# ds4dm/Tulip.jl

Measured on AMD Instinct MI355X. Metric: IPM Newton-step rate: KKT.update! (A*D*A'+Rd, supernodal Cholesky) + 4 KKT.solve!, higher is better.
Workload: dtype f64

## Files before the change

### tulip.jl_amd/csrc/kernels.hip

```cpp
#include <hip/hip_runtime.h>

#include <cstdlib>
#include <mutex>

#include "tlpk_device.hpp"

namespace tlpk {


typedef double v4f64 __attribute__((ext_vector_type(4)));
__device__ __forceinline__ double readlane_f64(const double v, const int l) {
    const int lo = __builtin_amdgcn_readlane(__double2loint(v), l), hi = __builtin_amdgcn_readlane(__double2hiint(v), l);
    return __hiloint2double(hi, lo);
}

__device__ __forceinline__ double *front_u(const DevCtx &c, const FrontDesc &fd) {
    return (fd.ubuf ? c.U1 : c.U0) + fd.uoff;
}
__device__ __forceinline__ double *pcol(const DevCtx &c, const FrontDesc &fd, i32 col) { return c.Lval + fd.loff + pk_off(fd.lda, col); }
__device__ __forceinline__ i32 pld(const FrontDesc &fd, i32 col) { return fd.lda - ((col >> 6) << 6); }

__global__ void k_compute_d(i64 n, const double *__restrict__ theta, const double *__restrict__ regP,
                            double *__restrict__ D) {
    const i64 j = (i64)blockIdx.x * blockDim.x + threadIdx.x;
// ... 1910 lines not shown
                any |= valid[a][b];
            }
    }
    v4f64 acc[CA][4];
#pragma unroll
    for (int a = 0; a < CA; ++a)
#pragma unroll
        for (int b = 0; b < 4; ++b) acc[a][b] = (v4f64){0.0, 0.0, 0.0, 0.0};

    const int lr = lane & 15, lk = lane >> 4;
    const int sr = tid & 127, sk0 = tid >> 7;
    const i32 ra = t.i0 + sr, rb_ = t.j0 + sr;
    const bool raok = FULL || (ra < f), rbok = FULL || ((rb_ < f) && !diag_tile);
    const int sk0u = __builtin_amdgcn_readfirstlane(sk0);
    double pa[UPD_NLD], pb[UPD_NLD];

    auto load_slab = [&](i32 kk, bool full_k) {
        if (FULL && full_k) {
#pragma unroll
            for (int it = 0; it < UPD_NLD; ++it) {
                const double *Pk = P + pk_off(lda, t.k0 + kk + sk0u + KS * it);
                pa[it] = Pk[ra];
                pb[it] = Pk[rb_];
                if (SIGNED) pb[it] *= sgk[kk + sk0 + KS * it];
            }
        } else {
#pragma unroll
            for (int it = 0; it < UPD_NLD; ++it) {
                const bool kok = (kk + sk0u + KS * it) < t.kw;
                const double *Pk = P + pk_off(lda, t.k0 + min(kk + sk0u + KS * it, t.kw - 1));
                pa[it] = (kok && raok) ? Pk[ra] : 0.0;
                pb[it] = (kok && rbok) ? Pk[rb_] : 0.0;
                if (SIGNED) pb[it] *= sgk[min(kk + sk0 + KS * it, t.kw - 1)];
            }
        }
    };
    auto store_slab = [&](int buf) {
#pragma unroll
        for (int it = 0; it < UPD_NLD; ++it) {
            const int k = sk0 + KS * it;
            As[buf][k * UPD_LD + sr] = pa[it];
            if (FULL || !diag_tile) Bs[buf][k * UPD_LD + sr] = pb[it];
        }
    };

    const i32 *segp = t.seg ? c.upd_seg + (t.seg - 1) : nullptr;
    if (segp || t.kw >= 2 * UPD_KT) {
        unsigned voa = (unsigned)min(t.i0 + sr, f - 1) * 8u, vob = (unsigned)min(t.j0 + sr, f - 1) * 8u;
        const char *Pc = reinterpret_cast<const char *>(P);
        const i32 nseg = __builtin_amdgcn_readfirstlane(segp ? segp[0] : 1);
        i32 k_slab = __builtin_amdgcn_readfirstlane(segp ? segp[1] : t.k0);
        i32 k_rem = __builtin_amdgcn_readfirstlane(segp ? segp[2] : (t.kw / UPD_KT));
        i32 k_seg = 0;
        const char *sb[UPD_NLD];
#pragma unroll
        for (int it = 0; it < UPD_NLD; ++it) sb[it] = Pc + pk_off(lda, k_slab + sk0u + KS * it) * 8;
        i64 step = (i64)UPD_KT * 8 * (lda - ((k_slab >> 6) << 6));
        auto ld_a = [&]() {
            asm volatile("" : "+v"(voa));
#pragma unroll
            for (int it = 0; it < UPD_NLD; ++it) pa[it] = *reinterpret_cast<const double *>(sb[it] + voa);
        };
        const double *sgf = SIGNED ? c.csign + fd.col0 : nullptr;
        auto ld_b = [&]() {
            asm volatile("" : "+v"(vob));
#pragma unroll
            for (int it = 0; it < UPD_NLD; ++it) {
                pb[it] = *reinterpret_cast<const double *>(sb[it] + vob);
                if (SIGNED) pb[it] *= sgf[k_slab + sk0 + KS * it];
            }
            k_slab += UPD_KT;
            const bool cross = (k_slab & 63) == 0;
#pragma unroll
            for (int it = 0; it < UPD_NLD; ++it) sb[it] += step - (cross ? (i64)(64 * 8) * (sk0u + KS * it + 1) : 0);
            step -= cross ? 64 * 8 * UPD_KT : 0;
            if (__builtin_expect(--k_rem == 0, 0)) {
                if (++k_seg < nseg) {
                    k_slab = __builtin_amdgcn_readfirstlane(segp[1 + 2 * k_seg]);
                    k_rem = __builtin_amdgcn_readfirstlane(segp[2 + 2 * k_seg]);
#pragma unroll
                    for (int it = 0; it < UPD_NLD; ++it) sb[it] = Pc + pk_off(lda, k_slab + sk0u + KS * it) * 8;
                    step = (i64)UPD_KT * 8 * (lda - ((k_slab >> 6) << 6));
                }
            }
        };
        auto st_ab = [&](int buf) {
#pragma unroll
            for (int it = 0; it < UPD_NLD; ++it) {
                As[buf][(sk0 + KS * it) * UPD_LD + sr] = pa[it];
                Bs[buf][(sk0 + KS * it) * UPD_LD + sr] = pb[it];
            }
        };
        auto mfma_round = [&](int buf, auto &&hook) {
            const double *At = As[buf] + wr * 64 + lr + lk * UPD_LD;
            const double *Bt = Bs[buf] + wc * WCW + lr + lk * UPD_LD;
#pragma unroll
            for (int k4 = 0; k4 < UPD_KT; k4 += 4) {
                double av[CA], bv[4];
                if (any) {
#pragma unroll
                    for (int a = 0; a < CA; ++a) av[a] = Bt[k4 * UPD_LD + a * 16];
#pragma unroll
                    for (int b = 0; b < 4; ++b) bv[b] = At[k4 * UPD_LD + b * 16];
                }
                hook(k4);
                if (any) {
#pragma unroll
                    for (int a = 0; a < CA; ++a)
#pragma unroll
                        for (int b = 0; b < 4; ++b)
                            acc[a][b] = __builtin_amdgcn_mfma_f64_16x16x4f64(av[a], bv[b], acc[a][b], 0, 0, 0);
                }
            }
        };
        int cur = 0;
        const i32 nrounds = segp ? t.nsl : t.kw / UPD_KT;
        const bool dma_ok = UPD_DMA && !SIGNED && ((fd.loff | (i64)lda | (i64)t.i0 | (i64)t.j0) & 1) == 0;
        if (dma_ok) {
            typedef __attribute__((address_space(3))) double upd_lds_double;
            const unsigned la_a0 = (unsigned)__builtin_amdgcn_readfirstlane((int)(unsigned)(unsigned long long)(upd_lds_double *)&As[0][0]);
            const unsigned la_b0 = (unsigned)__builtin_amdgcn_readfirstlane((int)(unsigned)(unsigned long long)(upd_lds_double *)&Bs[0][0]);
            constexpr unsigned BUFB = UPD_KT * UPD_LD * 8;
            constexpr int CPW = UPD_KT / NW;
            unsigned dva = (unsigned)min(t.i0 + 2 * lane, lda - 2) * 8u, dvb = (unsigned)min(t.j0 + 2 * lane, lda - 2) * 8u;
            const char *db[CPW];
#pragma unroll
            for (int e = 0; e < CPW; ++e) db[e] = Pc + pk_off(lda, k_slab + wave + NW * e) * 8;
            auto dma_slab = [&](const int buf) {
                asm volatile("" : "+v"(dva), "+v"(dvb));
#pragma unroll
                for (int e = 0; e < CPW; ++e) {
                    const unsigned ko = (unsigned)(wave + NW * e) * (unsigned)(UPD_LD * 8) + (unsigned)buf * BUFB;
                    asm volatile("s_mov_b32 m0, %0\n\ts_nop 0\n\tglobal_load_lds_dwordx4 %1, %2" :: "s"(la_a0 + ko), "v"(dva), "s"(db[e]) : "memory", "m0");
                    asm volatile("s_mov_b32 m0, %0\n\ts_nop 0\n\tglobal_load_lds_dwordx4 %1, %2" :: "s"(la_b0 + ko), "v"(dvb), "s"(db[e]) : "memory", "m0");
                }
                k_slab += UPD_KT;
                const bool cross = (k_slab & 63) == 0;
#pragma unroll
                for (int e = 0; e < CPW; ++e) db[e] += step - (cross ? (i64)(64 * 8) * (wave + NW * e + 1) : 0);
                step -= cross ? 64 * 8 * UPD_KT : 0;
                if (__builtin_expect(--k_rem == 0, 0)) {
                    if (++k_seg < nseg) {
                        k_slab = __builtin_amdgcn_readfirstlane(segp[1 + 2 * k_seg]);
                        k_rem = __builtin_amdgcn_readfirstlane(segp[2 + 2 * k_seg]);
#pragma unroll
                        for (int e = 0; e < CPW; ++e) db[e] = Pc + pk_off(lda, k_slab + wave + NW * e) * 8;
                        step = (i64)UPD_KT * 8 * (lda - ((k_slab >> 6) << 6));
                    }
                }
            };
            dma_slab(0);
            asm volatile("s_waitcnt vmcnt(0)" ::: "memory");
            __syncthreads();
            for (i32 rd = 0; rd < nrounds; ++rd) {
                const bool have_next = rd + 1 < nrounds;
                mfma_round(cur, [&](int k4) {
                    if (k4 == 0 && have_next) dma_slab(cur ^ 1);
                });
                asm volatile("s_waitcnt vmcnt(0)" ::: "memory");
                __syncthreads();
                cur ^= 1;
            }
        } else {
        ld_a(); ld_b();
        st_ab(0);
        ld_a(); ld_b();
        __syncthreads();
#ifdef UPD_TRACE
        if (threadIdx.x == 0) ((unsigned long long *)c.spart)[(size_t)blockIdx.x * 8 + 1] = wall_clock64();
#endif
        for (i32 rd = 0; rd < nrounds; ++rd) {
            const bool have_next = rd + 1 < nrounds, have_next2 = rd + 2 < nrounds;
            mfma_round(cur, [&](int k4) {
                if (k4 == 0 && have_next) st_ab(cur ^ 1);
                if (k4 == 4 && have_next2) ld_a();
                if (k4 == 8 && have_next2) ld_b();
            });
            __syncthreads();
            cur ^= 1;
        }
        }
        if (t.kw % UPD_KT) {
            const i32 kk = (t.kw / UPD_KT) * UPD_KT;
#pragma unroll
            for (int it = 0; it < UPD_NLD; ++it) {
                const bool kok = (kk + sk0u + KS * it) < t.kw;
                const double *Pk = P + pk_off(lda, t.k0 + min(kk + sk0u + KS * it, t.kw - 1));
                pa[it] = kok ? *reinterpret_cast<const double *>(reinterpret_cast<const char *>(Pk) + voa) : 0.0;
                pb[it] = kok ? *reinterpret_cast<const double *>(reinterpret_cast<const char *>(Pk) + vob) : 0.0;
                if (SIGNED) pb[it] *= sgk[min(kk + sk0 + KS * it, t.kw - 1)];
            }
            st_ab(cur);
            __syncthreads();
            mfma_round(cur, [](int) {});
        }
        goto epilogue;
    }
    {
    load_slab(0, UPD_KT <= t.kw);
    store_slab(0);
    __syncthreads();
    int cur = 0;
    for (i32 kk = 0; kk < t.kw; kk += UPD_KT) {
        const bool more = (kk + UPD_KT) < t.kw;
#if defined(UPD_VARIANT) && (UPD_VARIANT == 1 || UPD_VARIANT == 6)
        if (more && kk < 0) load_slab(kk + UPD_KT, true);
#else
        if (more) load_slab(kk + UPD_KT, (kk + 2 * UPD_KT) <= t.kw);
#endif
        if (any) {
            const double *At = As[cur] + wr * 64 + lr + lk * UPD_LD;
            const double *Bt = (diag_tile ? As[cur] : Bs[cur]) + wc * WCW + lr + lk * UPD_LD;
#pragma unroll
            for (int k4 = 0; k4 < UPD_KT; k4 += 4) {
                double av[CA], bv[4];
#pragma unroll
                for (int a = 0; a < CA; ++a) av[a] = Bt[k4 * UPD_LD + a * 16];
#pragma unroll
                for (int b = 0; b < 4; ++b) bv[b] = At[k4 * UPD_LD + b * 16];
#pragma unroll
                for (int a = 0; a < CA; ++a)
#pragma unroll
                    for (int b = 0; b < 4; ++b) {
                        if constexpr (FULL) {
                            acc[a][b] = __builtin_amdgcn_mfma_f64_16x16x4f64(av[a], bv[b], acc[a][b], 0, 0, 0);
                        } else {
                            if (valid[a][b]) acc[a][b] = __builtin_amdgcn_mfma_f64_16x16x4f64(av[a], bv[b], acc[a][b], 0, 0, 0);
                        }
                    }
            }
        }
        if (more) store_slab(cur ^ 1);
#if !(defined(UPD_VARIANT) && (UPD_VARIANT == 4 || UPD_VARIANT == 6))
        __syncthreads();
#endif
        cur ^= 1;
    }
    }
epilogue:
#ifdef UPD_TRACE
    if (threadIdx.x == 0) ((unsigned long long *)c.spart)[(size_t)blockIdx.x * 8 + 2] = wall_clock64();
#endif
    if (!any) return;
    if (t.pad1) {
        double *Sp = c.spart + (i64)(t.pad1 - 1) * (TILE * TILE);
#pragma unroll
        for (int a = 0; a < CA; ++a)
// ... 289 lines not shown

__device__ __forceinline__ bool chain_wait(const ChainItem &it, const unsigned *cnt, int *info, const int lane, const unsigned timeout_ms, const int dbg_slot) {
    const int n01 = it.n0 + it.n1, ntot = n01 + (it.w2 >= 0 ? 1 : 0);
    if (ntot == 0) return __hip_atomic_load(info + 1, __ATOMIC_RELAXED, __HIP_MEMORY_SCOPE_AGENT) == 0;
    const bool act = lane < ntot;
    const int e = min(lane, ntot - 1);
    const int idx = (e < it.n0) ? it.w0 + e : ((e < n01) ? it.w1 + (e - it.n0) : it.w2);
    const unsigned need = (unsigned)((e < it.n0) ? it.need0 : ((e < n01) ? it.need1 : it.need2));
    const unsigned *p = cnt + idx;
    bool dead = false;
    unsigned spins = 0;
    const unsigned long long t0 = wall_clock64();
    unsigned v = need;
    if (act) v = __hip_atomic_load(p, __ATOMIC_RELAXED, __HIP_MEMORY_SCOPE_AGENT);
    while (!dead && !__all(v >= need)) {
        if (spins < 64u) __builtin_amdgcn_s_sleep(8);
        else if (spins < 512u) __builtin_amdgcn_s_sleep(32);
        else __builtin_amdgcn_s_sleep(127);
        if ((++spins & 63u) == 0u) {
            int flag = 0;
            if (lane == 0) flag = __hip_atomic_load(info + 1, __ATOMIC_RELAXED, __HIP_MEMORY_SCOPE_AGENT);
            if (__builtin_amdgcn_readfirstlane(flag) != 0) dead = true;
            else if (wall_clock64() - t0 > (unsigned long long)timeout_ms * 100000ull) {
                if (v < need && __hip_atomic_exchange(info + 3, 1, __ATOMIC_RELAXED, __HIP_MEMORY_SCOPE_AGENT) == 0) {
                    info[4] = dbg_slot; info[5] = it.role; info[6] = idx; info[7] = (int)need; info[8] = (int)v; info[9] = (int)blockIdx.x; info[10] = (int)gridDim.x; info[11] = it.task;
                }
                if (lane == 0) __hip_atomic_store(info + 1, 1, __ATOMIC_RELAXED, __HIP_MEMORY_SCOPE_AGENT);
                dead = true;
            }
        }
        if (act) v = __hip_atomic_load(p, __ATOMIC_RELAXED, __HIP_MEMORY_SCOPE_AGENT);
    }
    asm volatile("" ::: "memory");
    __builtin_amdgcn_fence(__ATOMIC_ACQUIRE, "agent");
    return !dead;
}


template <class T> __device__ __forceinline__ T *uni(T *p) {
    const unsigned long long v = reinterpret_cast<unsigned long long>(p);
    const unsigned lo = (unsigned)__builtin_amdgcn_readfirstlane((int)(unsigned)v), hi = (unsigned)__builtin_amdgcn_readfirstlane((int)(unsigned)(v >> 32));
    typedef __attribute__((address_space(1))) T gT;
    return (T *)(gT *)(((unsigned long long)hi << 32) | lo);
}
typedef __attribute__((address_space(3))) double lds_double;
typedef __attribute__((address_space(3))) char lds_char;
__device__ __forceinline__ double *uni_lds(lds_double *p) {
    const unsigned v = (unsigned)__builtin_amdgcn_readfirstlane((int)(unsigned)(unsigned long long)(lds_char *)p);
    return (double *)(lds_double *)(lds_char *)(unsigned long long)v;
}
__device__ __forceinline__ DevCtx uni_ctx(const DevCtx &c) {
    DevCtx u = c;
    u.fronts = uni(c.fronts); u.Lval = uni(c.Lval); u.U0 = uni(c.U0); u.U1 = uni(c.U1); u.dinv = uni(c.dinv); u.spart = uni(c.spart); u.info = uni(c.info);
    u.csign = uni(c.csign); u.upd_seg = uni(c.upd_seg);
    return u;
}

template <bool SIGNED>
__device__ __noinline__ void chain_role_update(const UpdateTask *tp_, const DevCtx &c_, lds_double *lds_) {
    const UpdateTask *tp = uni(tp_); const DevCtx c = uni_ctx(c_); double *lds = uni_lds(lds_);
    const UpdateTask t{tp->front, tp->k0, tp->kw, tp->i0, tp->j0, tp->jlim, tp->beta0, tp->pad1, tp->seg, tp->nsl, tp->pad2, 0};
    const FrontDesc fd = c.fronts[t.front];
    if (t.pad2 == 2) { update_tile32<SIGNED>(t, fd, c); return; }
    if (t.pad2) { update_tile64<SIGNED>(t, fd, c, lds); return; }
    double (*As)[UPD_KT * UPD_LD] = reinterpret_cast<double (*)[UPD_KT * UPD_LD]>(lds);
    const bool full = (t.i0 + TILE <= fd.f) && (t.j0 + TILE <= t.jlim) && (t.i0 >= t.j0 + TILE);
    if (full) update_tile<true, SIGNED, 4>(t, fd, c, As, As + 2);
    else update_tile<false, SIGNED, 4>(t, fd, c, As, As + 2);
}
template <bool SIGNED>
__device__ __noinline__ void chain_role_potrf(const PotrfTask *tp_, const DevCtx &c_, lds_double *lds_, unsigned *prog_) {
    const PotrfTask *tp = uni(tp_); const DevCtx c = uni_ctx(c_); double *lds = uni_lds(lds_);
    const PotrfTask t{tp->front, tp->k0, tp->nb, tp->kprev};
    const FrontDesc fd = c.fronts[t.front];
    potrf_wide_task<SIGNED, 3>(t, fd, c, lds, prog_ ? uni(prog_) : nullptr);
    __builtin_amdgcn_s_setprio(0);
}
template <bool SIGNED>
__device__ __noinline__ void chain_role_trsm(const TrsmTask *tp_, const DevCtx &c_, lds_double *lds_, lds_double *dyn_, unsigned *cnt_, const unsigned timeout_ms_) {
    const TrsmTask *tp = uni(tp_); const DevCtx c = uni_ctx(c_); double *lds = uni_lds(lds_);
    const TrsmTask t{tp->front, tp->k0, tp->nb, tp->row0, tp->kprev, tp->fuse_nb, tp->pad1, tp->pad2};
    const FrontDesc fd = c.fronts[t.front];
    if (t.nb == NB_OUT) {
        if constexpr (TRSM_DMA) {
            const TrsmProg pg{t.pad2 > 0 ? uni(cnt_) + (t.pad2 - 1) : nullptr, c.info, (unsigned)__builtin_amdgcn_readfirstlane((int)timeout_ms_)};
            if (dyn_) {
                if (t.pad2 > 0) trsm_task_dma<SIGNED, 4, true>(t, fd, c, lds, uni_lds(dyn_), pg);
                else trsm_task_dma<SIGNED, 4, false>(t, fd, c, lds, uni_lds(dyn_), pg);
            } else {
                if (t.pad2 > 0) trsm_task_dma<SIGNED, 2, true>(t, fd, c, lds, nullptr, pg);
                else trsm_task_dma<SIGNED, 2, false>(t, fd, c, lds, nullptr, pg);
            }
        } else trsm_task<SIGNED, true>(t, fd, c, reinterpret_cast<double (*)[NB_IN * LDW]>(lds));
    } else trsm_task<SIGNED, false>(t, fd, c, reinterpret_cast<double (*)[NB_IN * LDW]>(lds));
}
__device__ __noinline__ void chain_role_reduce(const UpdateTask *tp_, const int sub_, const DevCtx &c_) {
    const UpdateTask *tp = uni(tp_); const DevCtx c = uni_ctx(c_); const int sub = __builtin_amdgcn_readfirstlane(sub_);
    const UpdateTask t{tp->front, tp->k0, tp->kw, tp->i0, tp->j0, tp->jlim, tp->beta0, tp->pad1, tp->seg, tp->nsl, 0, 0};
    const FrontDesc fd = c.fronts[t.front];
    reduce_part(t, sub, fd, c);
}

template <bool SIGNED>
__global__ __launch_bounds__(256, 2) void k_chain(const ChainArgs a, DevCtx c) {
    __shared__ __attribute__((aligned(16))) double lds[CHAIN_LDS];
    extern __shared__ __attribute__((aligned(16))) double chain_dyn[];
    lds_double *dyn = a.dyn_lds >= 2u * TRSM_DMA_BLK * sizeof(double) ? (lds_double *)chain_dyn : (lds_double *)nullptr;
// ... 1176 lines not shown
```

### tulip.jl_amd/csrc/tlpk_api.cpp

```cpp
#include <hip/hip_runtime.h>

#include <dlfcn.h>

#include <algorithm>
#include <atomic>
#include <chrono>
#include <climits>
#include <cmath>
#include <limits>
#include <cstdio>
#include <cstdlib>
#include <cstring>
#include <new>
#include <optional>
#include <string>
#include <thread>
#include <utility>
#include <vector>
#include <condition_variable>
#include <functional>
#include <initializer_list>
#include <mutex>

#include "../../include/tlpk.h"
// ... 249 lines not shown
            for (char f : S.front_fa) any_fa |= (f != 0);
            std::vector<i64> colptr_c;
            if (!every) {
                colptr_c.assign((size_t)S.m + 1, 0);
                i64 cnt = 0;
                for (i64 kk = 0; kk < S.m; ++kk) {
                    colptr_c[(size_t)kk] = cnt;
                    for (i64 e = S.Sp[(size_t)kk]; e < S.Sp[(size_t)kk + 1]; ++e) cnt += (S.s_local[(size_t)e] != 0);
                }
                colptr_c[(size_t)S.m] = cnt;
                if (cnt != d.n_asm) { h->last_error = "assembly list: column pointers do not match the compacted entries"; return TLPK_INTERNAL; }
            }
            const std::vector<i64> &colptr = every ? S.Sp : colptr_c;
            if (any_fa) {
                std::vector<i64> tsmall;
                if (every) tsmall.assign(S.s_target.begin(), S.s_target.end()); else tsmall = tgt;
                for (i64 kk = 0; kk < S.m; ++kk)
                    if (S.front_fa[(size_t)S.sn_of_col[(size_t)kk]])
                        for (i64 q = colptr[(size_t)kk]; q < colptr[(size_t)kk + 1]; ++q) tsmall[(size_t)q] = -1;
                UP(d.asm_colptr, colptr); UP(d.asm_target_small, tsmall);
            }
            bool any = false;
            for (char f : S.front_upper) any |= (f != 0);
            d.has_upper = any;
            if (any) {
                std::vector<unsigned char> up((size_t)d.n_asm, 0);
                for (i64 kk = 0; kk < S.m; ++kk)
                    if (S.front_upper[(size_t)S.sn_of_col[(size_t)kk]]) std::fill(up.begin() + colptr[(size_t)kk], up.begin() + colptr[(size_t)kk + 1], (unsigned char)1);
                UP(d.asm_upper, up);
            }
        }
        if (every) { UP(d.asm_target, S.s_target); UP(d.asm_diag, S.s_diag_row); UP(d.asm_ptr, S.pair_ptr); }
        else { UP(d.asm_target, tgt); UP(d.asm_diag, diag); UP(d.asm_ptr, ptr); }
        if (!d.asm_target_small) d.asm_target_small = d.asm_target;
        UP(d.pair_w, S.pair_w); UP(d.pair_j, S.pair_j);
        if (np != (i64)S.pair_w.size()) { h->last_error = "assembly list compaction mismatch"; return TLPK_INTERNAL; }
    }
    const FrontDesc *fr = nullptr; const i32 *ri = nullptr, *re = nullptr, *ch = nullptr;
    { FrontDesc *p; UP(p, S.fronts); fr = p; }
    { i32 *p; UP(p, S.rowidx); ri = p; }
    { i32 *p; UP(p, S.rel); re = p; }
    { i32 *p; UP(p, S.ea_tab); d.ctx.ea_tab = p; }
    { i32 *p; UP(p, S.children); ch = p; }
    d.ctx.fronts = fr; d.ctx.rowidx = ri; d.ctx.rel = re; d.ctx.children = ch;
    { i64 *p; UP(p, S.gth_ptr); d.ctx.gth_ptr = p; }
    { i64 *p; UP(p, S.gth_src); d.ctx.gth_src = p; }
    UP(d.fa_tasks, S.fa_tasks);
    UP(d.ea_tasks, S.ea_tasks); UP(d.potrf_tasks, S.potrf_tasks); UP(d.trsm_tasks, S.trsm_tasks);
    UP(d.update_tasks, S.update_tasks); UP(d.reduce_tasks, S.reduce_tasks);
    UP(d.chain_items, S.chain_items); d.n_chain_cnt = S.chain_counters;
    if (S.chain_counters > 0 && (rc = dev_alloc(h, &d.chain_cnt, S.chain_counters)) != TLPK_OK) return rc;
    if (!S.chain_items.empty() && std::getenv("TLPK_CHAIN_TRACE") && (rc = dev_alloc(h, &d.chain_trace, 4 * (i64)S.chain_items.size())) != TLPK_OK) return rc;
    { i32 *p; UP(p, S.upd_seg); d.ctx.upd_seg = p; }
    d.n_single = (i64)S.single_col.size();
    UP(d.single_loff, S.single_loff); UP(d.single_dinvoff, S.single_dinvoff); UP(d.single_col, S.single_col);
    UP(d.zero_tasks, S.zero_tasks); d.n_zero_tasks = (i64)S.zero_tasks.size() / 2; d.n_zero_lower = d.has_upper ? S.n_zero_lower : d.n_zero_tasks;
    UP(d.zero_small, S.zero_small); d.n_zero_small = (i64)S.zero_small.size();
    UP(d.fwd_gather_tasks, S.fwd_gather_tasks); UP(d.fwd_diag_tasks, S.fwd_diag_tasks);
    UP(d.fwd_update_tasks, S.fwd_update_tasks); UP(d.bwd_update_tasks, S.bwd_update_tasks);
    UP(d.fwd_small_tasks, S.fwd_small_tasks); UP(d.bwd_small_tasks, S.bwd_small_tasks);
    UP(d.fwd_sweep_tasks, S.fwd_sweep_tasks); UP(d.bwd_sweep_tasks, S.bwd_sweep_tasks);
#undef UP
#define AL(dst, cnt) if ((rc = dev_alloc(h, &(dst), (cnt))) != TLPK_OK) return rc
    AL(d.ctx.Lval, S.lval_len); AL(d.ctx.U0, S.ubuf_len[0]); AL(d.ctx.U1, S.ubuf_len[1]);
    if (std::getenv("TLPK_POISON") && S.lval_len > 0) { HIPCHK(h, hipMemset(d.ctx.Lval, 0xFF, (size_t)S.lval_len * 8)); HIPCHK(h, hipDeviceSynchronize()); }
    AL(d.ctx.uc, 2 * S.uc_len); AL(d.ctx.xw, 2 * S.m); AL(d.ctx.info, 16);
    d.ctx.xw2 = S.m; d.ctx.uc2 = S.uc_len; AL(d.ctx.dinv, S.dinv_len); AL(d.ctx.spart, S.spart_len);
    const i64 nn = std::max<i64>(S.n + (S.n_dense > 0 ? 1 : 0), S.k2_n + 1);
    AL(h->d_theta, nn); AL(h->d_regP, nn); AL(h->d_regD, S.m); AL(h->d_D, nn);
    AL(h->d_xip, S.m); AL(h->d_xid, nn); AL(h->d_dx, nn); AL(h->d_dy, S.m);
    AL(d.rhs_w, std::max<i64>(2 * S.n, 1));
    d.asm_D = h->d_D; d.asm_regD = h->d_regD;
    HIPCHK(h, hipMemset(h->d_theta, 0, (size_t)nn * 8)); HIPCHK(h, hipMemset(h->d_regP, 0, (size_t)nn * 8)); HIPCHK(h, hipMemset(h->d_xid, 0, (size_t)nn * 8));
    HIPCHK(h, hipMemset(h->d_regD, 0, (size_t)std::max<i64>(S.m, 1) * 8)); HIPCHK(h, hipMemset(h->d_xip, 0, (size_t)std::max<i64>(S.m, 1) * 8));
    if (h->refine_steps > 0) { AL(h->d_r1, S.m); AL(h->d_r2, nn); AL(h->d_cx, nn); AL(h->d_cy, S.m); AL(h->d_ref, 8); }
    d.ctx.csign = nullptr;
    d.ctx.small_full = std::getenv("TLPK_SMALL_FULL") ? std::atoi(std::getenv("TLPK_SMALL_FULL")) : 0;
    d.ctx.upd_remap = 2;
    if (const char *e = std::getenv("TLPK_UPD_REMAP")) d.ctx.upd_remap = std::atoi(e);
    if (S.system == 1 || S.n_dense > 0) { double *p; if ((rc = dev_upload(h, &p, S.csign)) != TLPK_OK) return rc; d.ctx.csign = p; }
#undef AL
    {
        i32 nslots = 0;
        h->sweep_slot_fwd.assign(S.fwd_launches.size(), -1); h->sweep_slot_bwd.assign(S.bwd_launches.size(), -1);
        for (size_t i = 0; i < S.fwd_launches.size(); ++i) if (S.fwd_launches[i].kind == LK_FWD_SWEEP) h->sweep_slot_fwd[i] = nslots++;
        for (size_t i = 0; i < S.bwd_launches.size(); ++i) if (S.bwd_launches[i].kind == LK_BWD_SWEEP) h->sweep_slot_bwd[i] = nslots++;
        const i64 nt = ((i64)nslots + 15) / 16 * 16;
        unsigned long long *blk = nullptr;
        if ((rc = dev_alloc(h, &blk, nt + 4 * S.m)) != TLPK_OK) return rc;
        d.sweep_tickets = blk; d.sweep_xh = reinterpret_cast<double *>(blk + nt);
        d.sweep_reset_bytes = (nt + 2 * S.m) * 8; d.sweep_reset_bytes2 = (nt + 4 * S.m) * 8;
        HIPCHK(h, hipMemset(d.ctx.info, 0, 16 * sizeof(int)));
    }
    HIPCHK(h, hipHostMalloc((void **)&h->h_info, 4 * sizeof(int), hipHostMallocDefault));
    h->h_info[0] = h->h_info[1] = h->h_info[2] = h->h_info[3] = 0;
    uvec<double>().swap(S.pair_w); uvec<i32>().swap(S.pair_j);
    return TLPK_OK;
}

void find_markers(tlpk_handle *h) {
    h->factor_marker = h->S.factor_launches.size();
    h->fwd_marker = h->S.fwd_launches.size();
    for (size_t i = 0; i < h->S.factor_launches.size(); ++i)
        if (h->S.factor_launches[i].kind == LK_ALLREDUCE_ROOT) h->factor_marker = i;
    for (size_t i = 0; i < h->S.fwd_launches.size(); ++i)
        if (h->S.fwd_launches[i].kind == LK_ALLREDUCE_ROOT) h->fwd_marker = i;
}

struct GraphKey { int kind; const void *p[8]; bool operator==(const GraphKey &o) const { return kind == o.kind && std::memcmp(p, o.p, sizeof(p)) == 0; } };

inline bool graph_usable(const tlpk_handle *h) {
    return h->use_graph && !h->profile && !h->serial && (h->S.ngroups <= 1 || h->force_graph);
}

inline bool graph_usable_solve(const tlpk_handle *h) {
    static const bool on = [] { const char *e = std::getenv("TLPK_GRAPH_SOLVE"); return e && std::atoi(e) != 0; }();
    if (graph_usable(h)) return true;
    return on && h->use_graph && !h->profile && !h->serial && h->S.solve_single_stream && !h->root_pending && h->opt.nranks == 1;
}

template <class F>
int graph_or_direct(tlpk_handle *h, const GraphKey &key, F &&body, bool usable) {
    if (!usable) return body();
    for (size_t i = 0; i < h->graph_keys.size(); ++i)
        if (*reinterpret_cast<const GraphKey *>(h->graph_keys[i].data()) == key) {
            HIPCHK(h, hipGraphLaunch(h->graph_execs[i], h->stream));
            return TLPK_OK;
        }
    hipGraph_t g = nullptr;
    if (hipStreamBeginCapture(h->stream, hipStreamCaptureModeThreadLocal) != hipSuccess) { (void)hipGetLastError(); h->use_graph = false; return body(); }
    const int rc = body();
    hipGraphExec_t exec = nullptr;
// ... 226 lines not shown
    if (rc == TLPK_OK) {
        find_markers(h);
        h->nlink = (h->S.root_front >= 0) ? h->S.fronts[h->S.root_front].ns : 0;
        h->first_link = h->S.m - h->nlink;
    }
    return rc;
}

static int create_device(tlpk_handle *h, const tlpk_options &def) {
    int rc = TLPK_OK;
    if (def.device >= 0) {
        int ndev = 0;
        if (hipGetDeviceCount(&ndev) != hipSuccess || def.device >= ndev) {
            h->last_error = "no HIP device " + std::to_string(def.device) + " visible";
            return TLPK_NO_DEVICE;
        }
        h->device = def.device;
        hipError_t e = hipSetDevice(h->device);
        if (e == hipSuccess) e = hipStreamCreateWithFlags(&h->stream, hipStreamNonBlocking);
        h->gstream[0] = h->stream;
        const int ng = std::max(1, h->S.ngroups);
        for (int g = 1; g < ng && e == hipSuccess; ++g) e = hipStreamCreateWithFlags(&h->gstream[g], hipStreamNonBlocking);
        for (int g = 0; g < ng && e == hipSuccess; ++g) e = hipStreamCreateWithFlags(&h->sstream[g], hipStreamNonBlocking);
        if (e == hipSuccess) e = hipEventCreateWithFlags(&h->ev_fork, hipEventDisableTiming);
        if (e == hipSuccess && ng >= 2) {
            int least = 0, greatest = 0;
            hipDeviceGetStreamPriorityRange(&least, &greatest);
            e = hipStreamCreateWithPriority(&h->zstream, hipStreamNonBlocking, least);
        }
        if (e == hipSuccess && ng >= 2) e = hipEventCreateWithFlags(&h->ev_zfork, hipEventDisableTiming);
        if (e == hipSuccess && ng >= 2) e = hipEventCreateWithFlags(&h->ev_upper, hipEventDisableTiming);
        for (int g = 1; g < ng && e == hipSuccess; ++g) e = hipEventCreateWithFlags(&h->ev_join[g], hipEventDisableTiming);
        for (int g = 0; g < ng && e == hipSuccess; ++g) e = hipEventCreateWithFlags(&h->ev_side[g], hipEventDisableTiming);
        if (e == hipSuccess && h->stagger) e = hipEventCreateWithFlags(&h->ev_stagger, hipEventDisableTiming);
        if (e == hipSuccess) e = hipEventCreate(&h->ev0);
        if (e == hipSuccess) e = hipEventCreate(&h->ev1);
        if (e == hipSuccess && h->S.root_front >= 0 && h->opt.nranks == 1) {
            e = hipStreamCreateWithFlags(&h->rstream, hipStreamNonBlocking);
            if (e == hipSuccess) e = hipEventCreateWithFlags(&h->ev_blocks, hipEventDisableTiming);
            if (e == hipSuccess) e = hipEventCreateWithFlags(&h->ev_root, hipEventDisableTiming);
        }
        if (e != hipSuccess) rc = hip_fail(h, e, "device init");
        if (rc == TLPK_OK) {
            size_t free_b = 0, total_b = 0;
            hipMemGetInfo(&free_b, &total_b);
            const double budget = def.mem_budget_bytes > 0 ? (double)def.mem_budget_bytes : 0.9 * (double)free_b;
            const double need = 8.0 * ((double)h->S.lval_len + (double)h->S.ubuf_len[0] + (double)h->S.ubuf_len[1] +
                                       (double)h->S.spart_len + (double)h->S.dinv_len + (double)h->S.uc_len +
                                       (double)h->S.gth_ptr.size() + (double)h->S.gth_src.size()) +
                                12.0 * (double)h->S.pair_w.size() + 21.0 * (double)h->S.nnzS + 52.0 * (double)h->S.nnzA +
                                8.0 * (double)h->S.rowidx.size() +
                                (double)sizeof(UpdateTask) * (double)(h->S.update_tasks.size() + h->S.reduce_tasks.size()) +
                                (double)sizeof(EaTask) * (double)h->S.ea_tasks.size() + (double)sizeof(TrsmTask) * (double)h->S.trsm_tasks.size() +
                                4.0 * (double)h->S.upd_seg.size() + 32.0 * (double)h->S.m;
            if (h->krylov) {
                rc = krylov_gate(h, budget);
            } else if (h->S.dense_matrix) {
                const double need_d = 8.0 * ((double)h->S.n * (double)dense_lda(h->S.m) + (double)h->S.lval_len + (double)h->S.spart_len + (double)h->S.dinv_len +
                                             2.0 * (double)h->S.gemv_chunks * (double)dense_lda(h->S.m) + 8.0 * (double)h->S.n + 12.0 * (double)h->S.m) +
                                      (double)sizeof(UpdateTask) * (double)(h->S.update_tasks.size() + h->S.reduce_tasks.size()) +
                                      (double)sizeof(TrsmTask) * (double)h->S.trsm_tasks.size() + (double)sizeof(ChainItem) * (double)h->S.chain_items.size();
                if (need_d > budget) {
                    h->last_error = "dense matrix: the device copy of A (" + std::to_string(8.0 * (double)h->S.n * (double)dense_lda(h->S.m)) + " bytes), the panel (" +
                                    std::to_string(8.0 * (double)h->S.lval_len) + " bytes) and the workspace need " + std::to_string((long long)need_d) +
                                    " bytes, budget " + std::to_string((long long)budget) + " bytes";
                    rc = TLPK_TOO_LARGE;
                }
            } else if (need > budget) {
                h->last_error = "factor needs " + std::to_string(need / 1e9) + " GB, budget " + std::to_string(budget / 1e9) + " GB";
                if (h->S.system == 0 && !h->S.Ap.empty()) {
                    i64 cmax = 0, jmax = -1;
                    for (i64 j = 0; j < h->S.n; ++j) { const i64 cj = h->S.Ap[(size_t)j + 1] - h->S.Ap[(size_t)j]; if (cj > cmax) { cmax = cj; jmax = j; } }
                    if (cmax >= 1000 && (double)cmax * (double)cmax >= 0.05 * (double)h->S.nnzL)
                        h->last_error += "; column " + std::to_string(jmax) + " of A has " + std::to_string(cmax) + " entries (a dense column fills the normal equations): "
                                         "the augmented system KKT_System = K2 (TLPK_SYSTEM_K2) does not form A*D*A'" +
                                         std::string(def.dense_cols == 0 ? "; or keep K1 with dense_cols = 1" : "");
                }
                rc = TLPK_TOO_LARGE;
            }
        }
        if (rc == TLPK_OK) rc = upload_all(h);
        if (rc == TLPK_OK && h->krylov) rc = krylov_upload(h);
        if (rc == TLPK_OK) h->has_device = true;
    } else if (def.mem_budget_bytes > 0 && h->krylov) {
        rc = krylov_gate(h, (double)def.mem_budget_bytes);
    } else if (def.mem_budget_bytes > 0) {
        const double need = 8.0 * ((double)h->S.lval_len + (double)h->S.ubuf_len[0] + (double)h->S.ubuf_len[1] +
                                   (h->S.dense_matrix ? (double)h->S.n * (double)dense_lda(h->S.m) + (double)h->S.spart_len : 0.0));
        if (need > (double)def.mem_budget_bytes) {
            h->last_error = "factor exceeds mem_budget_bytes";
            if (h->S.dense_matrix) h->last_error += ": " + std::to_string((long long)need) + " bytes needed (the device copy of A, the panel, the split-K scratch), budget " + std::to_string((long long)def.mem_budget_bytes) + " bytes";
            rc = TLPK_TOO_LARGE;
        }
    }
    return rc;
}

int tlpk_create(tlpk_handle **out, int64_t m, int64_t n, const int64_t *colptr, const int64_t *rowval,
                const double *nzval, int index_base, const tlpk_options *uopt) {
    if (!out) return TLPK_BADARG;
    *out = nullptr;
    tlpk_options def;
    tlpk_default_options(&def);
    if (uopt) {
        if (uopt->struct_size != (int32_t)sizeof(tlpk_options)) return TLPK_BADARG;
        def = *uopt;
    }
// ... 1596 lines not shown
    return TLPK_OK;
}

int64_t tlpk_symbolic_get(const tlpk_handle *h, const char *what, int64_t *buf, int64_t cap) {
    if (!h || !what) return -1;
    if (!h->sub.empty() && std::string(what) != "chain_retries") return tlpk_symbolic_get(h->sub[0], what, buf, cap);
    const Symbolic &S = h->S;
    std::vector<i64> tmp;
    const std::string w(what);
    auto from32 = [&](const auto &v) { tmp.assign(v.begin(), v.end()); };
    auto field = [&](auto getter) { tmp.resize(S.fronts.size()); for (size_t s = 0; s < S.fronts.size(); ++s) tmp[s] = (i64)getter(S.fronts[s]); };
    if (w == "perm") from32(S.perm);
    else if (w == "etree") from32(S.parent);
    else if (w == "colcount") from32(S.colcount);
    else if (w == "s_colptr") tmp = S.Sp;
    else if (w == "s_rowidx") from32(S.Si);
    else if (w == "s_target") from32(S.s_target);
    else if (w == "s_diag_row") from32(S.s_diag_row);
    else if (w == "pair_ptr") from32(S.pair_ptr);
    else if (w == "pair_j") from32(S.pair_j);
    else if (w == "rowidx") from32(S.rowidx);
    else if (w == "rel") from32(S.rel);
    else if (w == "ea_tab") from32(S.ea_tab);
    else if (w == "front_eatab") field([](const FrontDesc &f) { return f.eatab; });
    else if (w == "children") from32(S.children);
    else if (w == "depth") from32(S.depth);
    else if (w == "front_block") from32(S.front_block);
    else if (w == "row_block") tmp = h->row_block_copy;
    else if (w == "front_group") from32(S.front_group);
    else if (w == "ngroups") tmp.assign(1, S.ngroups);
    else if (w == "front_local") tmp.assign(S.front_local.begin(), S.front_local.end());
    else if (w == "col_local") tmp.assign(S.col_local.begin(), S.col_local.end());
    else if (w == "row_local") tmp.assign(S.row_local.begin(), S.row_local.end());
    else if (w == "front_f") field([](const FrontDesc &f) { return f.f; });
    else if (w == "front_lda") field([](const FrontDesc &f) { return f.lda; });
    else if (w == "front_ns") field([](const FrontDesc &f) { return f.ns; });
    else if (w == "front_col0") field([](const FrontDesc &f) { return f.col0; });
    else if (w == "front_parent") field([](const FrontDesc &f) { return f.parent; });
    else if (w == "front_loff") field([](const FrontDesc &f) { return f.loff; });
    else if (w == "front_rowoff") field([](const FrontDesc &f) { return f.rowoff; });
    else if (w == "front_reloff") field([](const FrontDesc &f) { return f.reloff; });
    else if (w == "front_child_ptr") field([](const FrontDesc &f) { return f.child_ptr; });
    else if (w == "front_nchild") field([](const FrontDesc &f) { return f.nchild; });
    else if (w == "root_front") tmp.assign(1, S.root_front);
    else if (w == "dense_cols") tmp = S.dense_cols;
    else if (w == "potrf_tasks") { for (auto &t : S.potrf_tasks) { tmp.push_back(t.front); tmp.push_back(t.k0); tmp.push_back(t.nb); tmp.push_back(t.kprev); } }
    else if (w == "trsm_tasks") { for (auto &t : S.trsm_tasks) { tmp.push_back(t.front); tmp.push_back(t.k0); tmp.push_back(t.nb); tmp.push_back(t.row0); tmp.push_back(t.kprev); tmp.push_back(t.pad1); } }
    else if (w == "update_tasks") { for (auto &t : S.update_tasks) { tmp.push_back(t.front); tmp.push_back(t.k0); tmp.push_back(t.kw); tmp.push_back(t.i0); tmp.push_back(t.j0); tmp.push_back(t.jlim); tmp.push_back(t.beta0); tmp.push_back(t.pad1); tmp.push_back(t.seg); tmp.push_back(t.nsl); } }
    else if (w == "upd_seg") from32(S.upd_seg);
    else if (w == "trsm_early") { for (auto &t : S.trsm_tasks) tmp.push_back(t.pad2); }
    else if (w == "update_tile64") { for (auto &t : S.update_tasks) tmp.push_back(t.pad2); }
    else if (w == "skip_off") tmp = S.skip_off;
    else if (w == "skip_bits") { tmp.resize(S.skip_bits.size()); std::memcpy(tmp.data(), S.skip_bits.data(), S.skip_bits.size() * 8); }
    else if (w == "front_single") tmp.assign(S.front_single.begin(), S.front_single.end());
    else if (w == "reduce_tasks") { for (auto &t : S.reduce_tasks) { tmp.push_back(t.front); tmp.push_back(t.k0); tmp.push_back(t.kw); tmp.push_back(t.i0); tmp.push_back(t.j0); tmp.push_back(t.jlim); tmp.push_back(t.beta0); tmp.push_back(t.pad1); } }
    else if (w == "chain_items") { for (auto &t : S.chain_items) { for (i32 v : {t.role, t.task, t.sub, t.w0, t.n0, t.need0, t.w1, t.n1, t.need1, t.w2, t.need2, t.sig}) tmp.push_back(v); } }
    else if (w == "chain_counters") tmp.assign(1, S.chain_counters);
    else if (w == "krylov_unsolved") tmp.assign(1, h->krylov_unsolved);
    else if (w == "chain_retries") tmp.assign(1, h->chain_retries);
    else if (w == "chain_trace") {
        if (!h->d.chain_trace) return -1;
        tmp.resize(4 * S.chain_items.size());
        if (hipMemcpy(tmp.data(), h->d.chain_trace, tmp.size() * 8, hipMemcpyDeviceToHost) != hipSuccess) return -1;
    }
    else if (w == "fa_tasks") { for (auto &t : S.fa_tasks) { tmp.push_back(t.front); tmp.push_back(t.bc); tmp.push_back(t.br0); tmp.push_back(t.br1); } }
    else if (w == "front_fa") tmp.assign(S.front_fa.begin(), S.front_fa.end());
    else if (w == "front_upper") tmp.assign(S.front_upper.begin(), S.front_upper.end());
    else if (w == "ea_tasks") { for (auto &t : S.ea_tasks) { tmp.push_back(t.front); tmp.push_back(t.j0); tmp.push_back(t.j1); tmp.push_back(t.bidx); tmp.push_back(t.br0); tmp.push_back(t.br1); } }
    else if (w == "fwd_gather_tasks" || w == "fwd_diag_tasks" || w == "fwd_update_tasks" || w == "bwd_update_tasks" || w == "fwd_small_tasks" || w == "bwd_small_tasks" ||
             w == "fwd_sweep_tasks" || w == "bwd_sweep_tasks") {
        const std::vector<SolveTask> &v = (w == "fwd_gather_tasks") ? S.fwd_gather_tasks : (w == "fwd_diag_tasks") ? S.fwd_diag_tasks :
                                          (w == "fwd_update_tasks") ? S.fwd_update_tasks : (w == "bwd_update_tasks") ? S.bwd_update_tasks :
                                          (w == "fwd_small_tasks") ? S.fwd_small_tasks : (w == "bwd_small_tasks") ? S.bwd_small_tasks :
                                          (w == "fwd_sweep_tasks") ? S.fwd_sweep_tasks : S.bwd_sweep_tasks;
        for (auto &t : v) { tmp.push_back(t.front); tmp.push_back(t.k0); tmp.push_back(t.nb); tmp.push_back(t.row0); tmp.push_back(t.slot); tmp.push_back(t.nslot); }
    }
    else if (w == "front_flagoff") field([](const FrontDesc &f) { return f.flagoff; });
    else if (w == "n_sweep_flags") tmp.assign(1, S.n_sweep_flags);
    else if (w == "front_ucoff") field([](const FrontDesc &f) { return f.ucoff; });
    else if (w == "front_uoff") field([](const FrontDesc &f) { return f.uoff; });
    else if (w == "front_ubuf") field([](const FrontDesc &f) { return f.ubuf; });
    else if (w == "gth_ptr") tmp.assign(S.gth_ptr.begin(), S.gth_ptr.end());
    else if (w == "gth_src") tmp.assign(S.gth_src.begin(), S.gth_src.end());
    else if (w == "factor_launches") { for (auto &L : S.factor_launches) { tmp.push_back(L.kind); tmp.push_back(L.first); tmp.push_back(L.count); } }
    else if (w == "fwd_launches") { for (auto &L : S.fwd_launches) { tmp.push_back(L.kind); tmp.push_back(L.first); tmp.push_back(L.count); } }
    else if (w == "bwd_launches") { for (auto &L : S.bwd_launches) { tmp.push_back(L.kind); tmp.push_back(L.first); tmp.push_back(L.count); } }
    else if (w == "launch_meta") { for (auto *v : {&S.factor_launches, &S.fwd_launches, &S.bwd_launches}) for (auto &L : *v) { tmp.push_back(L.group); tmp.push_back(L.side); tmp.push_back(L.pad); } }
    else if (w == "zero_tasks") from32(S.zero_tasks);
    else if (w == "zero_small") from32(S.zero_small);
    else if (w == "singles") {
        tmp = S.single_loff; tmp.insert(tmp.end(), S.single_dinvoff.begin(), S.single_dinvoff.end()); tmp.insert(tmp.end(), S.single_col.begin(), S.single_col.end());
        tmp.push_back(S.n_zero_lower); tmp.push_back(S.spart_len);
    }
    else return -1;
    const i64 len = (i64)tmp.size();
    if (buf) std::copy(tmp.begin(), tmp.begin() + std::min(len, cap), buf);
    return len;
}

int64_t tlpk_symbolic_get_f64(const tlpk_handle *h, const char *what, double *buf, int64_t cap) {
    if (!h || !what) return -1;
    const std::string w(what);
    if (w != "pair_w") return -1;
    const auto &v = h->S.pair_w;
    i64 len = (i64)v.size();
    if (len == 0 && h->values_set && h->sub.empty() && h->has_device && h->d.pair_w && !h->S.pair_ptr.empty()) {
// ... 42 lines not shown
```

### tulip.jl_amd/csrc/tlpk_device.hpp

```cpp
#pragma once
#include <hip/hip_runtime.h>

#include "tlpk_host.hpp"

namespace tlpk {

struct DevCtx {
    const FrontDesc *fronts;
    const i32 *rowidx;
    const i32 *rel;
    const i32 *ea_tab;
    const i32 *children;
    const i64 *gth_ptr, *gth_src;
    double *Lval;
    double *U0, *U1;
    double *uc;
    double *xw;
    double *dinv;
    double *spart;
    int *info;
    int upd_remap;
    const double *csign;
    const i32 *upd_seg;
    int small_full;
    i64 xw2, uc2;
};

struct SweepArgs {
    unsigned long long *ticket;
    double *xh;
    i64 xh2;
    int poll_fast, poll_nfast, poll_slow;
    const SolveTask *small = nullptr;
};

struct DevArrays {
    DevCtx ctx{};
    i64 m = 0, n = 0;
    i64 mu = 0;
    char *sparse_col = nullptr; i32 *dense_col = nullptr; i64 n_dense = 0;
    const double *dA = nullptr; i64 dlda = 0;
    i32 syrk_split = 1; i64 syrk_kc = 0;
    double *gemv_part = nullptr; i64 gemv_chunks = 0, gemv_cw = 0;
    i64 *Ap = nullptr; i32 *Ai = nullptr; double *Ax = nullptr;
    i64 *Tp = nullptr; i32 *Tj = nullptr; double *Tx = nullptr;
    i32 *perm = nullptr;
    i64 *Pp = nullptr; i32 *Pj = nullptr; double *Px = nullptr;
    double *rhs_w = nullptr;
    i32 *zero_tasks = nullptr; i64 n_zero_tasks = 0;
    i64 n_zero_lower = 0;
    unsigned char *asm_upper = nullptr; bool has_upper = false;
    i32 *zero_small = nullptr; i64 n_zero_small = 0;
    char *row_local = nullptr, *col_local = nullptr;
    i64 n_asm = 0;
    i64 *asm_target = nullptr; i32 *asm_diag = nullptr; i64 *asm_ptr = nullptr;
    double *pair_w = nullptr; i32 *pair_j = nullptr;
    FaTask *fa_tasks = nullptr;
    i64 *asm_colptr = nullptr;
    i64 *asm_target_small = nullptr;
    const double *asm_D = nullptr, *asm_regD = nullptr;
    EaTask *ea_tasks = nullptr; PotrfTask *potrf_tasks = nullptr; TrsmTask *trsm_tasks = nullptr;
    UpdateTask *update_tasks = nullptr, *reduce_tasks = nullptr;
    ChainItem *chain_items = nullptr;
    unsigned long long *chain_trace = nullptr;
    unsigned *chain_cnt = nullptr; i64 n_chain_cnt = 0;
    i64 n_single = 0; i64 *single_loff = nullptr, *single_dinvoff = nullptr; i32 *single_col = nullptr;
    SolveTask *fwd_gather_tasks = nullptr, *fwd_diag_tasks = nullptr, *fwd_update_tasks = nullptr,
              *bwd_update_tasks = nullptr, *fwd_small_tasks = nullptr, *bwd_small_tasks = nullptr,
              *fwd_sweep_tasks = nullptr, *bwd_sweep_tasks = nullptr;
    unsigned long long *sweep_tickets = nullptr;
    double *sweep_xh = nullptr;
    i64 sweep_reset_bytes = 0, sweep_reset_bytes2 = 0;
};

void launch_compute_d(hipStream_t st, i64 n, const double *theta, const double *regP, double *D);
void launch_assemble(hipStream_t st, const DevArrays &a, const double *D, const double *regD, int part = -1);
void launch_zero_panels(hipStream_t st, const DevArrays &a, int part = -1);
void launch_tasks(hipStream_t st, const DevArrays &a, const Launch &L, const SweepArgs *sw = nullptr, int nrhs = 1);
// ... 117 lines not shown
```

Before: 20.40.

## Skip MFMA rounds per wave when skip-bitmap shows zero update slabs

Adds a per-wave skip test in the supernodal update GEMM kernel. It reads a precomputed sparsity bitmap (skip_bits/skip_off) for each 16-column k-slab and the wave's row and column windows. When either side is structurally zero, the wave skips the LDS reads and MFMAs for that round. The bitmap words are loaded a round or two ahead through scalar constant-address loads, and a small queue tracks the decisions. This removes wasted MFMA work on zero blocks, at the cost of extra scalar loads and bookkeeping, and it is on by default via an env flag.

```diff
diff --git a/tulip.jl_amd/csrc/kernels.hip b/tulip.jl_amd/csrc/kernels.hip
--- a/tulip.jl_amd/csrc/kernels.hip
+++ b/tulip.jl_amd/csrc/kernels.hip
@@ -1986,6 +1986,27 @@
         i32 k_slab = __builtin_amdgcn_readfirstlane(segp ? segp[1] : t.k0);
         i32 k_rem = __builtin_amdgcn_readfirstlane(segp ? segp[2] : (t.kw / UPD_KT));
         i32 k_seg = 0;
+        const i64 ws_off = c.upd_wave_skip ? c.skip_off[t.front] : (i64)-1;
+        typedef __attribute__((address_space(4))) const uint32_t ws_word;
+        const ws_word *ws_bits = ws_off >= 0 ? (const ws_word *)(unsigned long long)(c.skip_bits + ws_off) : nullptr;
+        const i32 ws_w2 = (i32)(2 * skip_words(f));
+        SkipWin ws_a = (SkipWin)__builtin_amdgcn_readfirstlane((int)skip_window(f, ibase, 64)), ws_b = (SkipWin)__builtin_amdgcn_readfirstlane((int)skip_window(f, jbase, WCW));
+        unsigned ws_q = 0;
+        uint64_t ws_va = 0, ws_vb = 0;
+        auto ws_load = [&]() {
+            if (ws_bits) {
+                const ws_word *row = ws_bits + (i64)(k_slab >> 4) * ws_w2;
+                ws_va = skip_window_load(row, ws_a); ws_vb = skip_window_load(row, ws_b);
+            }
+        };
+        auto ws_request = [&](const int ahead) {
+            unsigned need = 1;
+            if (ws_bits) {
+                const bool na = skip_window_test(ws_va, ws_a), nb = skip_window_test(ws_vb, ws_b);
+                need = (unsigned)__builtin_amdgcn_readfirstlane((int)(na & nb));
+            }
+            ws_q |= need << ahead;
+        };
         const char *sb[UPD_NLD];
 #pragma unroll
         for (int it = 0; it < UPD_NLD; ++it) sb[it] = Pc + pk_off(lda, k_slab + sk0u + KS * it) * 8;
@@ -2003,6 +2024,7 @@
                 pb[it] = *reinterpret_cast<const double *>(sb[it] + vob);
                 if (SIGNED) pb[it] *= sgf[k_slab + sk0 + KS * it];
             }
+            ws_request(2);
             k_slab += UPD_KT;
             const bool cross = (k_slab & 63) == 0;
 #pragma unroll
@@ -2025,20 +2047,22 @@
                 Bs[buf][(sk0 + KS * it) * UPD_LD + sr] = pb[it];
             }
         };
-        auto mfma_round = [&](int buf, auto &&hook) {
+        auto mfma_round = [&](int buf, const bool need, auto &&pre, auto &&hook) {
             const double *At = As[buf] + wr * 64 + lr + lk * UPD_LD;
             const double *Bt = Bs[buf] + wc * WCW + lr + lk * UPD_LD;
+            const bool run = any & need;
 #pragma unroll
             for (int k4 = 0; k4 < UPD_KT; k4 += 4) {
                 double av[CA], bv[4];
-                if (any) {
+                pre(k4);
+                if (run) {
 #pragma unroll
                     for (int a = 0; a < CA; ++a) av[a] = Bt[k4 * UPD_LD + a * 16];
 #pragma unroll
                     for (int b = 0; b < 4; ++b) bv[b] = At[k4 * UPD_LD + b * 16];
                 }
                 hook(k4);
-                if (any) {
+                if (run) {
 #pragma unroll
                     for (int a = 0; a < CA; ++a)
 #pragma unroll
@@ -2068,6 +2092,7 @@
                     asm volatile("s_mov_b32 m0, %0\n\ts_nop 0\n\tglobal_load_lds_dwordx4 %1, %2" :: "s"(la_a0 + ko), "v"(dva), "s"(db[e]) : "memory", "m0");
                     asm volatile("s_mov_b32 m0, %0\n\ts_nop 0\n\tglobal_load_lds_dwordx4 %1, %2" :: "s"(la_b0 + ko), "v"(dvb), "s"(db[e]) : "memory", "m0");
                 }
+                ws_request(1);
                 k_slab += UPD_KT;
                 const bool cross = (k_slab & 63) == 0;
 #pragma unroll
@@ -2083,33 +2108,42 @@
                     }
                 }
             };
-            dma_slab(0);
+            ws_load(); dma_slab(0);
+            ws_q >>= 1;
             asm volatile("s_waitcnt vmcnt(0)" ::: "memory");
             __syncthreads();
             for (i32 rd = 0; rd < nrounds; ++rd) {
                 const bool have_next = rd + 1 < nrounds;
-                mfma_round(cur, [&](int k4) {
+                mfma_round(cur, (ws_q & 1u) != 0, [&](int k4) {
+                    if (k4 == 0 && have_next) ws_load();
+                }, [&](int k4) {
                     if (k4 == 0 && have_next) dma_slab(cur ^ 1);
                 });
+                ws_q >>= 1;
                 asm volatile("s_waitcnt vmcnt(0)" ::: "memory");
                 __syncthreads();
                 cur ^= 1;
             }
         } else {
-        ld_a(); ld_b();
+        ws_load(); ld_a(); ld_b();
+        ws_q >>= 1;
         st_ab(0);
-        ld_a(); ld_b();
+        ws_load(); ld_a(); ld_b();
+        ws_q >>= 1;
         __syncthreads();
 #ifdef UPD_TRACE
         if (threadIdx.x == 0) ((unsigned long long *)c.spart)[(size_t)blockIdx.x * 8 + 1] = wall_clock64();
 #endif
         for (i32 rd = 0; rd < nrounds; ++rd) {
             const bool have_next = rd + 1 < nrounds, have_next2 = rd + 2 < nrounds;
-            mfma_round(cur, [&](int k4) {
+            mfma_round(cur, (ws_q & 1u) != 0, [&](int k4) {
+                if (k4 == 8 && have_next2) ws_load();
+            }, [&](int k4) {
                 if (k4 == 0 && have_next) st_ab(cur ^ 1);
                 if (k4 == 4 && have_next2) ld_a();
                 if (k4 == 8 && have_next2) ld_b();
             });
+            ws_q >>= 1;
             __syncthreads();
             cur ^= 1;
         }
@@ -2126,7 +2160,7 @@
             }
             st_ab(cur);
             __syncthreads();
-            mfma_round(cur, [](int) {});
+            mfma_round(cur, true, [](int) {}, [](int) {});
         }
         goto epilogue;
     }
@@ -2522,7 +2556,7 @@
 __device__ __forceinline__ DevCtx uni_ctx(const DevCtx &c) {
     DevCtx u = c;
     u.fronts = uni(c.fronts); u.Lval = uni(c.Lval); u.U0 = uni(c.U0); u.U1 = uni(c.U1); u.dinv = uni(c.dinv); u.spart = uni(c.spart); u.info = uni(c.info);
-    u.csign = uni(c.csign); u.upd_seg = uni(c.upd_seg);
+    u.csign = uni(c.csign); u.upd_seg = uni(c.upd_seg); u.skip_off = uni(c.skip_off); u.skip_bits = uni(c.skip_bits); u.upd_wave_skip = __builtin_amdgcn_readfirstlane(c.upd_wave_skip);
     return u;
 }
 
diff --git a/tulip.jl_amd/csrc/tlpk_api.cpp b/tulip.jl_amd/csrc/tlpk_api.cpp
--- a/tulip.jl_amd/csrc/tlpk_api.cpp
+++ b/tulip.jl_amd/csrc/tlpk_api.cpp
@@ -325,6 +325,8 @@
     if (S.chain_counters > 0 && (rc = dev_alloc(h, &d.chain_cnt, S.chain_counters)) != TLPK_OK) return rc;
     if (!S.chain_items.empty() && std::getenv("TLPK_CHAIN_TRACE") && (rc = dev_alloc(h, &d.chain_trace, 4 * (i64)S.chain_items.size())) != TLPK_OK) return rc;
     { i32 *p; UP(p, S.upd_seg); d.ctx.upd_seg = p; }
+    { i64 *p; UP(p, S.skip_off); d.ctx.skip_off = p; }
+    { uint64_t *p; UP(p, S.skip_bits); d.ctx.skip_bits = p; }
     d.n_single = (i64)S.single_col.size();
     UP(d.single_loff, S.single_loff); UP(d.single_dinvoff, S.single_dinvoff); UP(d.single_col, S.single_col);
     UP(d.zero_tasks, S.zero_tasks); d.n_zero_tasks = (i64)S.zero_tasks.size() / 2; d.n_zero_lower = d.has_upper ? S.n_zero_lower : d.n_zero_tasks;
@@ -351,6 +353,9 @@
     d.ctx.small_full = std::getenv("TLPK_SMALL_FULL") ? std::atoi(std::getenv("TLPK_SMALL_FULL")) : 0;
     d.ctx.upd_remap = 2;
     if (const char *e = std::getenv("TLPK_UPD_REMAP")) d.ctx.upd_remap = std::atoi(e);
+    d.ctx.upd_wave_skip = 1;
+    if (const char *e = std::getenv("TLPK_UPD_WAVE_SKIP")) d.ctx.upd_wave_skip = std::atoi(e) != 0;
+    if (S.skip_bits.empty()) d.ctx.upd_wave_skip = 0;
     if (S.system == 1 || S.n_dense > 0) { double *p; if ((rc = dev_upload(h, &p, S.csign)) != TLPK_OK) return rc; d.ctx.csign = p; }
 #undef AL
     {
@@ -683,7 +688,7 @@
                                 8.0 * (double)h->S.rowidx.size() +
                                 (double)sizeof(UpdateTask) * (double)(h->S.update_tasks.size() + h->S.reduce_tasks.size()) +
                                 (double)sizeof(EaTask) * (double)h->S.ea_tasks.size() + (double)sizeof(TrsmTask) * (double)h->S.trsm_tasks.size() +
-                                4.0 * (double)h->S.upd_seg.size() + 32.0 * (double)h->S.m;
+                                4.0 * (double)h->S.upd_seg.size() + 8.0 * (double)(h->S.skip_off.size() + h->S.skip_bits.size()) + 32.0 * (double)h->S.m;
             if (h->krylov) {
                 rc = krylov_gate(h, budget);
             } else if (h->S.dense_matrix) {
@@ -2386,6 +2391,29 @@
     else if (w == "update_tile64") { for (auto &t : S.update_tasks) tmp.push_back(t.pad2); }
     else if (w == "skip_off") tmp = S.skip_off;
     else if (w == "skip_bits") { tmp.resize(S.skip_bits.size()); std::memcpy(tmp.data(), S.skip_bits.data(), S.skip_bits.size() * 8); }
+    else if (w == "upd_wave_skip") {
+        for (auto &t : S.update_tasks) {
+            const FrontDesc &fd = S.fronts[(size_t)t.front];
+            const i64 off = S.skip_off[(size_t)t.front];
+            const bool decided = off >= 0 && t.pad2 == 0 && (t.seg || t.kw >= 32);
+            auto slab = [&](i32 kcol) {
+                i64 m8 = 0xFF, m4 = 0xF;
+                if (decided) {
+                    m8 = m4 = 0;
+                    const uint64_t *bits = S.skip_bits.data() + off;
+                    for (int wv = 0; wv < 8; ++wv) if (wave_computes_slab(bits, fd.f, kcol / 16, t.i0 + (wv >> 2) * 64, t.j0 + (wv & 3) * 32, 32)) m8 |= (i64)1 << wv;
+                    for (int wv = 0; wv < 4; ++wv) if (wave_computes_slab(bits, fd.f, kcol / 16, t.i0 + (wv >> 1) * 64, t.j0 + (wv & 1) * 64, 64)) m4 |= (i64)1 << wv;
+                }
+                tmp.push_back(m8); tmp.push_back(m4);
+            };
+            if (t.seg) {
+                const i32 *sp = S.upd_seg.data() + (t.seg - 1);
+                for (i32 q = 0; q < sp[0]; ++q) for (i32 e = 0; e < sp[2 + 2 * q]; ++e) slab(sp[1 + 2 * q] + 16 * e);
+            } else {
+                for (i32 e = 0; e < t.kw / 16; ++e) slab(t.k0 + 16 * e);
+            }
+        }
+    }
     else if (w == "front_single") tmp.assign(S.front_single.begin(), S.front_single.end());
     else if (w == "reduce_tasks") { for (auto &t : S.reduce_tasks) { tmp.push_back(t.front); tmp.push_back(t.k0); tmp.push_back(t.kw); tmp.push_back(t.i0); tmp.push_back(t.j0); tmp.push_back(t.jlim); tmp.push_back(t.beta0); tmp.push_back(t.pad1); } }
     else if (w == "chain_items") { for (auto &t : S.chain_items) { for (i32 v : {t.role, t.task, t.sub, t.w0, t.n0, t.need0, t.w1, t.n1, t.need1, t.w2, t.need2, t.sig}) tmp.push_back(v); } }
diff --git a/tulip.jl_amd/csrc/tlpk_device.hpp b/tulip.jl_amd/csrc/tlpk_device.hpp
--- a/tulip.jl_amd/csrc/tlpk_device.hpp
+++ b/tulip.jl_amd/csrc/tlpk_device.hpp
@@ -2,6 +2,7 @@
 #include <hip/hip_runtime.h>
 
 #include "tlpk_host.hpp"
+#include "upd_wave_skip.hpp"
 
 namespace tlpk {
 
@@ -24,6 +25,9 @@
     const i32 *upd_seg;
     int small_full;
     i64 xw2, uc2;
+    const i64 *skip_off;
+    const uint64_t *skip_bits;
+    int upd_wave_skip;
 };
 
 struct SweepArgs {
diff --git a/tulip.jl_amd/csrc/upd_wave_skip.hpp b/tulip.jl_amd/csrc/upd_wave_skip.hpp
--- /dev/null
+++ b/tulip.jl_amd/csrc/upd_wave_skip.hpp
@@ -0,0 +1,39 @@
+#pragma once
+#include <cstdint>
+
+#if defined(__HIPCC__) || defined(__CUDACC__)
+#define TLPK_HD __host__ __device__
+#else
+#define TLPK_HD
+#endif
+
+namespace tlpk {
+
+typedef uint32_t SkipWin;
+
+TLPK_HD inline int64_t skip_words(int32_t f) { return (((int64_t)f + 15) / 16 + 63) / 64; }
+
+TLPK_HD inline SkipWin skip_window(int32_t f, int32_t r0, int32_t n) {
+    const int32_t end = (r0 + n < f) ? r0 + n : f;
+    const int32_t g0 = r0 >> 4, g1 = (end - 1) >> 4, last = (int32_t)(2 * skip_words(f)) - 1;
+    if (g1 < g0) return 0;
+    const int32_t lo = (g0 >> 5) < last ? (g0 >> 5) : last - 1;
+    return ((uint32_t)lo << 10) | ((uint32_t)(g0 - 32 * lo) << 4) | (uint32_t)(g1 - g0 + 1);
+}
+
+template <class Row> TLPK_HD inline uint64_t skip_window_load(Row row, const SkipWin w) {
+    const uint32_t lo = w >> 10;
+    return ((uint64_t)row[lo + 1] << 32) | row[lo];
+}
+TLPK_HD inline bool skip_window_test(const uint64_t v, const SkipWin w) {
+    const uint32_t sh = (w >> 4) & 63u, cnt = w & 15u;
+    return ((v >> sh) & (((uint64_t)1 << cnt) - 1)) != 0;
+}
+template <class Row> TLPK_HD inline bool skip_window_any(Row row, const SkipWin w) { return skip_window_test(skip_window_load(row, w), w); }
+
+TLPK_HD inline bool wave_computes_slab(const uint64_t *bits, int32_t f, int32_t k, int32_t ra, int32_t rb, int32_t nb) {
+    const uint32_t *row = reinterpret_cast<const uint32_t *>(bits + (int64_t)k * skip_words(f));
+    return skip_window_any(row, skip_window(f, ra, 64)) && skip_window_any(row, skip_window(f, rb, nb));
+}
+
+}
```

After: 20.38. Within noise of the previous version (-0.1%).
